# thunguyenphuoc/RenderNet

Hardware: AMD Instinct MI355X
Metric: rendered frames/sec, 64^3 voxel->512x512 Phong, batch 24 (higher is better)
Workload: dtype f32 (multiply stages: bf16x3-split operands, fp32 accumulate); 1 GPU; Phong shader forward (resampler + RenderNet 1-ch head), 5 shipped binvox fixtures cycled, 64^3 -> 128^3 -> 512x512, seeded random weights (237.3M params); batch_per_gpu=24, global_batch=24

## Files before the change

### include/rendernet_hip.h

```cpp
#ifndef RENDERNET_HIP_H
#define RENDERNET_HIP_H

#include <stddef.h>
#include <stdint.h>

#ifdef __cplusplus
extern "C" {
#endif

#define RN_VERSION 193

#define RN_OK              0
#define RN_E_INVALID      -1
#define RN_E_LAUNCH       -2
#define RN_E_UNSUPPORTED  -3

#define RN_ACT_NONE     0
#define RN_ACT_PRELU    1
#define RN_ACT_SIGMOID  2
#define RN_ACT_ELU      4

#define RN_PACK_CONV        0
#define RN_PACK_CONVT_S1    1
#define RN_PACK_CONVT_S2    2
// ... 82 lines not shown
int rn_winograd_input_transform(int scheme, const float* x, float* V, int B, int H, int W, int C, int pad_lo, void* stream);
int rn_winograd_gemm(int scheme, const float* V, const float* w_packed, float* M, long long T, int Cin, int Cout, void* stream);
int rn_winograd_output_transform(int scheme, const float* M, const float* bias, const float* alpha, const float* residual,
                                 float* y, float* preact, int B, int H, int W, int C, int act, void* stream);
#define RN_SPLIT_FMT_H2 0x100
int rn_winograd_split_supported(int scheme, int Cin, int Cout);
size_t rn_winograd_split_packed_bytes(int scheme, int Cin, int Cout);
size_t rn_winograd_split_v_bytes(int scheme, long long T, int Cin);
size_t rn_winograd_split_workspace_bytes(int scheme, int B, int H, int W, int Cin, int Cout);
int rn_winograd_split_pack(int scheme, const float* w_tf, void* w_split, int Cin, int Cout, int transposed, void* stream);
int rn_winograd_split_input_transform(int scheme, const float* x, void* Vs, int B, int H, int W, int C, int pad_lo, void* stream);
int rn_winograd_split_gemm(int scheme, const void* Vs, const void* w_split, float* M, long long T, int Cin, int Cout, void* stream);
int rn_conv2d_winograd_split_fwd(int scheme, const float* x, const void* w_split, const float* bias, const float* alpha,
                                 const float* residual, float* y, float* preact, void* workspace, int B, int H, int W,
                                 int Cin, int Cout, int transposed, int act, void* stream);
int rn_conv2d_winograd_split_fwd_ex(int scheme, const float* x, const void* w_split, const float* bias, const float* alpha,
                                    const float* residual, float* y, float* preact, void* workspace, int B, int H, int W,
                                    int Cin, int Cout, int transposed, int act, const void* amax_x, void* amax_y, void* stream);
int rn_winograd_split_input_transform_ex(int scheme, const float* x, void* Vs, int B, int H, int W, int C, int pad_lo,
                                         const void* amax_x, void* stream);
int rn_winograd_output_transform_ex(int scheme, const float* M, const float* bias, const float* alpha, const float* residual,
                                    float* y, float* preact, int B, int H, int W, int C, int act, void* amax_y, void* stream);
int rn_absmax(const float* x, long long n, void* amax, void* stream);
int rn_winograd_split_wgrad_supported(int scheme, int Cin, int Cout);
size_t rn_winograd_split_wgrad_workspace_bytes(int scheme, int B, int H, int W, int Cin, int Cout);
int rn_conv2d_winograd_split_wgrad(int scheme, const float* x, const float* dz, float* dw, void* workspace, int B, int H, int W,
                                   int Cin, int Cout, void* stream);
int rn_conv3d_winograd_split_supported(int Cin, int Cout);
size_t rn_conv3d_winograd_split_packed_bytes(int Cin, int Cout);
int rn_conv3d_winograd_split_pack(const float* w_tf, void* w_split, int Cin, int Cout, int transposed, void* stream);
int rn_conv3d_winograd_split_fwd(const float* x, const void* w_split, const float* bias, const float* alpha, const float* residual,
                                 float* y, float* preact, int B, int H, int W, int D, int Cin, int Cout, int act, void* stream);
size_t rn_conv3d_winograd_split_packed_bytes_ex(int fmt, int Cin, int Cout);
int rn_conv3d_winograd_split_pack_ex(int fmt, const float* w_tf, void* w_split, int Cin, int Cout, int transposed, void* stream);
int rn_conv3d_winograd_split_fwd_ex(int fmt, const float* x, const void* w_split, const float* bias, const float* alpha, const float* residual,
                                    float* y, float* preact, int B, int H, int W, int D, int Cin, int Cout, int act,
                                    const void* amax_x, void* amax_scratch, void* amax_y, void* stream);
int rn_conv3d_wino_supported(int Cin, int Cout);
int rn_conv2d_wino4_supported(int Cin, int Cout);
int rn_conv2d_wino4_fwd(const float* x, const float* w_wino4, const float* bias, const float* alpha,
                        const float* residual, float* y, float* preact,
                        int B, int H, int W, int Cin, int Cout, int transposed, int act, void* stream);

int rn_conv2d_transpose_s2_wino_supported(int Cin, int Cout);
int rn_conv2d_transpose_s2_wino_fwd(const float* x, const float* w_wino_s2, const float* bias, const float* alpha,
                                    const float* residual, float* y, float* preact,
// ... 171 lines not shown
```

### rendernet_amd/_lib.py

```python
import ctypes
import os

_HERE = os.path.dirname(os.path.abspath(__file__))
LIB_PATH = os.environ.get("RN_HIP_LIBRARY") or os.path.join(_HERE, "lib", "librendernet_hip.so")

RN_ACT_NONE, RN_ACT_PRELU, RN_ACT_SIGMOID, RN_ACT_ELU = 0, 1, 2, 4
RN_PHONG_NP_BLACK, RN_PHONG_NP_WHITE, RN_PHONG_TF_BLACK, RN_PHONG_TF_WHITE, RN_PHONG_NO_MASK = 0, 1, 2, 3, 4
RN_PACK_CONV, RN_PACK_CONVT_S1, RN_PACK_CONVT_S2, RN_PACK_CONV_WINO, RN_PACK_CONVT_S1_WINO = 0, 1, 2, 3, 4
RN_PACK_CONV_WINO4, RN_PACK_CONVT_S1_WINO4 = 5, 6
RN_PACK_CONV_WINO43, RN_PACK_CONVT_S1_WINO43 = 7, 8
RN_PACK_CONV_WINO44, RN_PACK_CONVT_S1_WINO44 = 9, 10
RN_PACK_CONV_WINO63, RN_PACK_CONVT_S1_WINO63 = 11, 12
RN_PACK_CONVT_S2_WINO = 13
RN_WINO_F43, RN_WINO_F44, RN_WINO_F63, RN_WINO_F11 = 0, 1, 2, 3
RN_SHAPES_MAX_PRIMS, RN_SHAPES_NOOP = 8, 255
RN_METRICS_U8, RN_METRICS_F32 = 0, 1
RN_SPLIT_FMT_H2 = 0x100

_c_int, _c_vp, _c_f = ctypes.c_int, ctypes.c_void_p, ctypes.c_float
_ip = ctypes.POINTER(ctypes.c_int)

SIGNATURES = {
    "rn_version": (_c_int, []),
    "rn_last_error": (ctypes.c_char_p, []),
# ... 42 lines not shown
    "rn_conv2d_wino43_workspace_floats": (ctypes.c_size_t, [_c_int] * 5),
    "rn_conv2d_wino43_fwd": (_c_int, [_c_vp] * 8 + [_c_int] * 6 + [_c_vp]),
    "rn_conv2d_wino63_supported": (_c_int, [_c_int, _c_int]),
    "rn_conv2d_wino63_workspace_floats": (ctypes.c_size_t, [_c_int] * 5),
    "rn_conv2d_wino63_fwd": (_c_int, [_c_vp] * 8 + [_c_int] * 6 + [_c_vp]),
    "rn_conv2d_wino44_supported": (_c_int, [_c_int, _c_int]),
    "rn_conv2d_wino44_workspace_floats": (ctypes.c_size_t, [_c_int] * 5),
    "rn_conv2d_wino44_fwd": (_c_int, [_c_vp] * 8 + [_c_int] * 7 + [_c_vp]),
    "rn_winograd_input_transform": (_c_int, [_c_int, _c_vp, _c_vp] + [_c_int] * 5 + [_c_vp]),
    "rn_winograd_gemm": (_c_int, [_c_int] + [_c_vp] * 3 + [ctypes.c_longlong, _c_int, _c_int, _c_vp]),
    "rn_winograd_output_transform": (_c_int, [_c_int] + [_c_vp] * 6 + [_c_int] * 5 + [_c_vp]),
    "rn_winograd_split_supported": (_c_int, [_c_int] * 3),
    "rn_winograd_split_packed_bytes": (ctypes.c_size_t, [_c_int] * 3),
    "rn_winograd_split_v_bytes": (ctypes.c_size_t, [_c_int, ctypes.c_longlong, _c_int]),
    "rn_winograd_split_workspace_bytes": (ctypes.c_size_t, [_c_int] * 6),
    "rn_winograd_split_pack": (_c_int, [_c_int, _c_vp, _c_vp, _c_int, _c_int, _c_int, _c_vp]),
    "rn_winograd_split_input_transform": (_c_int, [_c_int, _c_vp, _c_vp] + [_c_int] * 5 + [_c_vp]),
    "rn_winograd_split_gemm": (_c_int, [_c_int] + [_c_vp] * 3 + [ctypes.c_longlong, _c_int, _c_int, _c_vp]),
    "rn_conv2d_winograd_split_fwd": (_c_int, [_c_int] + [_c_vp] * 8 + [_c_int] * 7 + [_c_vp]),
    "rn_conv2d_winograd_split_fwd_ex": (_c_int, [_c_int] + [_c_vp] * 8 + [_c_int] * 7 + [_c_vp] * 3),
    "rn_winograd_split_input_transform_ex": (_c_int, [_c_int, _c_vp, _c_vp] + [_c_int] * 5 + [_c_vp, _c_vp]),
    "rn_winograd_output_transform_ex": (_c_int, [_c_int] + [_c_vp] * 6 + [_c_int] * 5 + [_c_vp, _c_vp]),
    "rn_absmax": (_c_int, [_c_vp, ctypes.c_longlong, _c_vp, _c_vp]),
    "rn_winograd_split_wgrad_supported": (_c_int, [_c_int, _c_int, _c_int]),
    "rn_winograd_split_wgrad_workspace_bytes": (ctypes.c_size_t, [_c_int] * 6),
    "rn_conv2d_winograd_split_wgrad": (_c_int, [_c_int] + [_c_vp] * 4 + [_c_int] * 5 + [_c_vp]),
    "rn_conv3d_winograd_split_supported": (_c_int, [_c_int, _c_int]),
    "rn_conv3d_winograd_split_packed_bytes_ex": (ctypes.c_size_t, [_c_int, _c_int, _c_int]),
    "rn_conv3d_winograd_split_pack_ex": (_c_int, [_c_int, _c_vp, _c_vp, _c_int, _c_int, _c_int, _c_vp]),
    "rn_conv3d_winograd_split_fwd_ex": (_c_int, [_c_int] + [_c_vp] * 7 + [_c_int] * 7 + [_c_vp] * 4),
    "rn_conv3d_winograd_split_packed_bytes": (ctypes.c_size_t, [_c_int, _c_int]),
    "rn_conv3d_winograd_split_pack": (_c_int, [_c_vp, _c_vp, _c_int, _c_int, _c_int, _c_vp]),
    "rn_conv3d_winograd_split_fwd": (_c_int, [_c_vp] * 7 + [_c_int] * 7 + [_c_vp]),
    "rn_conv2d_wino43_wgrad_supported": (_c_int, [_c_int, _c_int]),
    "rn_conv2d_wino43_wgrad_workspace_floats": (ctypes.c_size_t, [_c_int] * 5),
    "rn_conv2d_wino43_wgrad": (_c_int, [_c_vp] * 4 + [_c_int] * 5 + [_c_vp]),
    "rn_conv2d_wino44_wgrad_supported": (_c_int, [_c_int, _c_int]),
    "rn_conv2d_wino44_wgrad_workspace_floats": (ctypes.c_size_t, [_c_int] * 5),
    "rn_conv2d_wino44_wgrad": (_c_int, [_c_vp] * 4 + [_c_int] * 5 + [_c_vp]),
    "rn_conv2d_wino_wgrad_supported": (_c_int, [_c_int, _c_int]),
    "rn_conv2d_wino_wgrad": (_c_int, [_c_vp] * 3 + [_c_int] * 5 + [_c_vp]),
    "rn_conv2d_transpose_wgrad": (_c_int, [_c_vp] * 3 + [_c_int] * 7 + [_c_vp]),
    "rn_conv3d_transpose_wgrad": (_c_int, [_c_vp] * 3 + [_c_int] * 8 + [_c_vp]),
    "rn_resample_affine_bwd": (_c_int, [_c_vp] * 5 + [_c_int] * 9 + [_c_vp]),
    "rn_pose_to_affine_bwd": (_c_int, [_c_vp] * 3 + [_c_int] * 3 + [_c_vp]),
    "rn_dropout": (_c_int, [_c_vp, _c_vp, ctypes.c_size_t, _c_f, ctypes.c_uint64, ctypes.c_uint64, _c_vp]),
# ... 49 lines not shown

def check(rc, what=""):
    if rc != 0:
        msg = lib().rn_last_error()
        raise RenderNetHipError("%s failed (rc=%d): %s" % (what, rc, msg.decode() if msg else ""))


def ivec(vals):
    return (ctypes.c_int * len(vals))(*[int(v) for v in vals])


def ptr(t):
    if t is None:
        return None
    if not t.is_cuda:
        raise RenderNetHipError("expected a CUDA/HIP tensor, got device %s" % t.device)
    if _F32[0] is None:
        lib()
    if t.dtype is not _F32[0] or not t.is_contiguous():
        raise RenderNetHipError("expected a contiguous float32 tensor")
    return ctypes.c_void_p(t.data_ptr())


def stream_ptr():
    import torch
    return ctypes.c_void_p(torch.cuda.current_stream().cuda_stream)
```

### rendernet_amd/csrc/capi.hip

```cpp
#include "rn_common.h"
#include <stdarg.h>
#include <stdio.h>

static thread_local char g_err[512] = "";

int rn_set_error(int code, const char* fmt, ...)
{
    va_list ap;
    va_start(ap, fmt);
    vsnprintf(g_err, sizeof(g_err), fmt, ap);
    va_end(ap);
    return code;
}

int rn_check_launch(const char* what)
{
    hipError_t e = hipGetLastError();
    if (e != hipSuccess) return rn_set_error(RN_E_LAUNCH, "%s: %s", what, hipGetErrorString(e));
    return RN_OK;
}

int rn_ensure_dynamic_lds(const void* kernel, size_t bytes)
{
    struct Slot { const void* k; int dev; size_t bytes; };
// ... 417 lines not shown
}
extern "C" size_t rn_winograd_split_workspace_bytes(int scheme, int B, int H, int W, int Cin, int Cout)
{
    if (B < 1 || H < 1 || W < 1 || !rn_wino_bf3_supported(scheme, Cin, Cout)) return 0;
    return rn_wino_bf3_workspace_bytes(scheme, B, H, W, Cin, Cout);
}
extern "C" int rn_winograd_split_pack(int scheme, const float* w_tf, void* w_split, int Cin, int Cout, int transposed, void* stream)
{
    if (!w_tf || !w_split) return rn_set_error(RN_E_INVALID, "rn_winograd_split_pack: null pointer");
    return rn_launch_wino_pack_bf3(scheme, w_tf, w_split, Cin, Cout, transposed ? 1 : 0, (hipStream_t)stream);
}
extern "C" int rn_winograd_split_input_transform(int scheme, const float* x, void* Vs, int B, int H, int W, int C, int pad_lo, void* stream)
{
    if (!x || !Vs) return rn_set_error(RN_E_INVALID, "rn_winograd_split_input_transform: null pointer");
    if (rn_split_scheme_nxi(scheme & 0xff) == 0 || (scheme >> 8) > 1 || B < 1 || H < 1 || W < 1 || C < 32 || C % 32 != 0 || pad_lo < 0 || pad_lo > 3)
        return rn_set_error(RN_E_INVALID, "rn_winograd_split_input_transform: bad arguments (C must be a multiple of 32: the GEMM stage's K contract)");
    return rn_launch_wino_input_bf3(scheme, x, Vs, B, H, W, C, pad_lo, (hipStream_t)stream);
}
extern "C" int rn_winograd_split_gemm(int scheme, const void* Vs, const void* w_split, float* M, long long T, int Cin, int Cout, void* stream)
{
    if (!Vs || !w_split || !M) return rn_set_error(RN_E_INVALID, "rn_winograd_split_gemm: null pointer");
    return rn_launch_wino_gemm_bf3(scheme, Vs, w_split, M, T, Cin, Cout, (hipStream_t)stream);
}
extern "C" int rn_conv2d_winograd_split_fwd(int scheme, const float* x, const void* w_split, const float* bias, const float* alpha,
                                            const float* residual, float* y, float* preact, void* workspace, int B, int H, int W,
                                            int Cin, int Cout, int transposed, int act, void* stream)
{
    if (!x || !w_split || !y || !workspace) return rn_set_error(RN_E_INVALID, "rn_conv2d_winograd_split_fwd: null pointer");
    if (B < 1 || H < 1 || W < 1) return rn_set_error(RN_E_INVALID, "rn_conv2d_winograd_split_fwd: bad sizes");
    if ((act & RN_ACT_PRELU) && !alpha) return rn_set_error(RN_E_INVALID, "rn_conv2d_winograd_split_fwd: PReLU needs alpha");
    const int pad_lo = (scheme & 0xff) == RN_WINO_F11 ? 0 : ((scheme & 0xff) == RN_WINO_F44 && transposed) ? 2 : 1;
    return rn_launch_conv_wino_bf3(scheme, x, w_split, bias, alpha, residual, y, preact, workspace, B, H, W, Cin, Cout, pad_lo, act,
                                   (hipStream_t)stream);
}

extern "C" int rn_conv2d_winograd_split_fwd_ex(int scheme, const float* x, const void* w_split, const float* bias, const float* alpha,
                                               const float* residual, float* y, float* preact, void* workspace, int B, int H, int W,
                                               int Cin, int Cout, int transposed, int act, const void* amax_x, void* amax_y, void* stream)
{
    if (!x || !w_split || !y || !workspace) return rn_set_error(RN_E_INVALID, "rn_conv2d_winograd_split_fwd_ex: null pointer");
    if (B < 1 || H < 1 || W < 1) return rn_set_error(RN_E_INVALID, "rn_conv2d_winograd_split_fwd_ex: bad sizes");
    if ((act & RN_ACT_PRELU) && !alpha) return rn_set_error(RN_E_INVALID, "rn_conv2d_winograd_split_fwd_ex: PReLU needs alpha");
    const int pad_lo = (scheme & 0xff) == RN_WINO_F11 ? 0 : ((scheme & 0xff) == RN_WINO_F44 && transposed) ? 2 : 1;
    return rn_launch_conv_wino_bf3_ex(scheme, x, w_split, bias, alpha, residual, y, preact, workspace, B, H, W, Cin, Cout, pad_lo, act,
                                      static_cast<const unsigned*>(amax_x), static_cast<unsigned*>(amax_y), (hipStream_t)stream);
}
// ... 182 lines not shown
```

### rendernet_amd/csrc/conv_wino43.hip

```cpp
#include "wino_xform.h"
#include <stdlib.h>

namespace {

constexpr int GBM = 256, GBN = 256, GBK = 32;
constexpr int G_UB = GBK * GBN * 4;

__device__ __forceinline__ f32x4 ld4(const float* p) { return *reinterpret_cast<const f32x4*>(p); }
__device__ __forceinline__ void st4(float* p, f32x4 v) { *reinterpret_cast<f32x4*>(p) = v; }

}

template <class S, int VW>
__global__ __launch_bounds__(256)
void wino_input_kernel(const float* __restrict__ x, float* __restrict__ V, int H, int W, int C, int th, int tw,
                       long long T, unsigned nblk8, int pad_lo)
{
    typedef float vec __attribute__((ext_vector_type(VW)));
    constexpr int A = S::TA;
    const unsigned blk = xcd_contiguous(blockIdx.x, nblk8);
    const long long idx = (long long)blk * 256 + threadIdx.x;
    const int CV = C / VW;
    const int cv = (int)(idx % CV);
    const long long t = idx / CV;
    if (t >= T) return;
    vec tt[A][A];
    wino_input_btd<S, BT_DENSE>(x, t, true, cv * VW, H, W, C, th, tw, pad_lo, tt);
    float* vb = V + (size_t)t * C + cv * VW;
    const size_t plane = (size_t)T * C;
#pragma unroll
    for (int i = 0; i < A; ++i) {
        vec vrow[A];
        bt_apply<S, BT_DENSE>(tt[i], vrow);
#pragma unroll
        for (int j = 0; j < A; ++j) *reinterpret_cast<vec*>(vb + (size_t)(i * A + j) * plane) = vrow[j];
    }
}

template <class S, int VW, bool RES = false>
__global__ __launch_bounds__(256)
void wino_output_kernel(const float* __restrict__ M, const float* __restrict__ bias, const float* __restrict__ alpha,
                        const float* __restrict__ res, float* __restrict__ y, float* __restrict__ z,
                        int H, int W, int C, int th, int tw, long long T, int act, unsigned nblk8, unsigned* __restrict__ amax)
{
    typedef float vec __attribute__((ext_vector_type(VW)));
    constexpr int A = S::TA;
    const unsigned blk = xcd_contiguous(blockIdx.x, nblk8);
    const long long idx = (long long)blk * 256 + threadIdx.x;
    const int CV = C / VW;
    const int cv = (int)(idx % CV);
    const long long t_raw = idx / CV;
    if (t_raw >= T && !amax) return;
    const bool live = t_raw < T;
    const long long t = live ? t_raw : T - 1;
    float ymax = 0.f;
    const int tx = (int)(t % tw), ty = (int)((t / tw) % th);
    const long long b = t / ((long long)tw * th);
    const float* mb = M + (size_t)t * C + cv * VW;
    const size_t plane = (size_t)T * C;
    constexpr int MO = S::M;
    vec s[MO][A];
#pragma unroll
    for (int j = 0; j < A; ++j) {
        vec m[A];
#pragma unroll
        for (int i = 0; i < A; ++i) m[i] = __builtin_nontemporal_load(reinterpret_cast<const vec*>(mb + (size_t)(i * A + j) * plane));
#pragma unroll
        for (int p_ = 0; p_ < MO; ++p_) {
            vec acc = vec(0.f);
#pragma unroll
            for (int i = 0; i < A; ++i) {
                const float c = S::AT(p_, i);
                if (c != 0.f) acc += c * m[i];
            }
            s[p_][j] = acc;
        }
    }
// ... 357 lines not shown
    if (ragged > 0) {
        a.mb_begin = full; a.mblocks = 1;
        const int nitems = nxi * a.nblocks;
        int best_wm = 4, best_parts = 1, best_cost = (nitems + 255) / 256 * 4;
        for (int wm = 2; wm >= 1; --wm) {
            const int parts = (ragged + wm * 64 - 1) / (wm * 64);
            const int cost = (nitems * parts + 255) / 256 * wm;
            if (cost < best_cost) { best_wm = wm; best_parts = parts; best_cost = cost; }
        }
        return wino43_gemm_launch(best_wm, tag, a, 0, nitems, best_parts, st);
    }
    return RN_OK;
}

int rn_launch_wino_output(int scheme, const float* M, const float* bias, const float* alpha, const float* residual, float* y,
                          float* preact, int B, int H, int W, int C, int act, hipStream_t st)
{
    return rn_launch_wino_output_amax(scheme, M, bias, alpha, residual, y, preact, B, H, W, C, act, nullptr, st);
}

int rn_launch_wino_output_amax(int scheme, const float* M, const float* bias, const float* alpha, const float* residual, float* y,
                               float* preact, int B, int H, int W, int C, int act, unsigned* amax, hipStream_t st)
{
    const int m = rn_split_scheme_m(scheme);
    if (m == 0) return rn_set_error(RN_E_INVALID, "wino_output: unknown scheme %d", scheme);
    const int th = (H + m - 1) / m, tw = (W + m - 1) / m;
    const long long T = (long long)B * th * tw;
    if (!wino_with_scheme<WINO_SPLIT>(scheme, [&](auto s) {
            typedef decltype(s) S;
            constexpr int VW = wino_vw<S>;
            const unsigned long long n = ((unsigned long long)T * (C / VW) + 255) / 256;
            const unsigned nblk8 = (unsigned)((n + 7) / 8 * 8);
            if (residual) hipLaunchKernelGGL((wino_output_kernel<S, VW, true>), dim3(nblk8), dim3(256), 0, st, M, bias, alpha, residual, y, preact,
                                             H, W, C, th, tw, T, act, nblk8, amax);
            else hipLaunchKernelGGL((wino_output_kernel<S, VW, false>), dim3(nblk8), dim3(256), 0, st, M, bias, alpha, residual, y, preact,
                                    H, W, C, th, tw, T, act, nblk8, amax);
        }))
        return rn_set_error(RN_E_INVALID, "wino_output: unknown scheme %d", scheme);
    return rn_check_launch("wino_output");
}

long long rn_wino43_plane_limit()
{
    const char* e = getenv("RN_WINO43_MAX_PLANE");
    const long long v = e ? atoll(e) : 0;
    return (v > 0 && v < 0x7fffff00LL) ? v : 0x7fffff00LL;
}

size_t rn_wino43_workspace_floats(int scheme, int B, int H, int W, int Cin, int Cout)
{
    const int m = rn_wino_scheme_m(scheme);
    if (m == 0) return 0;
    const size_t T = (size_t)B * ((H + m - 1) / m) * ((W + m - 1) / m);
    return (size_t)rn_wino_scheme_nxi(scheme) * T * ((size_t)Cin + Cout);
}

int rn_launch_conv_wino43(int scheme, const float* x, const float* u, const float* bias, const float* alpha, const float* residual,
                          float* y, float* preact, float* ws, int B, int H, int W, int Cin, int Cout, int pad_lo, int act, hipStream_t st)
{
// ... 28 lines not shown
```

### rendernet_amd/csrc/conv_wino_bf3.hip

```cpp
#include "wino_xform.h"
#include <stdlib.h>

#ifndef RN_BF3_M_AUX
#define RN_BF3_M_AUX 0
#endif
#ifndef RN_BF3_VLOAD_AUX
#define RN_BF3_VLOAD_AUX 0
#endif
#ifndef RN_BF3_ULOAD_AUX
#define RN_BF3_ULOAD_AUX 0
#endif
#ifndef RN_BF3_VSTORE_NT
#define RN_BF3_VSTORE_NT 0
#endif

using rnf::FmtB3;
using rnf::FmtH2;

namespace {
constexpr int SB_ROW = 96;
constexpr int SB_BM = 256, SB_BN = 256;
constexpr int SB_NSTAGE = 3;
}

// ... 666 lines not shown
    hipLaunchKernelGGL(kern, dim3(n < 256 ? (unsigned)((n + 7) / 8 * 8) : 256u), dim3(512), lds, st, a);
    return rn_check_launch("wino_gemm_bf3");
}

template <class F, int WM>
static int wino_gemm_bf3_launch_w(int tag, const Bf3GemmArgs& a, int begin, int end, int parts, hipStream_t st)
{
    switch (tag) {
    case 0: return wino_gemm_bf3_launch_t<F, WM, 0>(a, begin, end, parts, st);
    case 1: return wino_gemm_bf3_launch_t<F, WM, 1>(a, begin, end, parts, st);
    case 2: return wino_gemm_bf3_launch_t<F, WM, 2>(a, begin, end, parts, st);
    case 4: return wino_gemm_bf3_launch_t<F, WM, 4>(a, begin, end, parts, st);
    case 5: return wino_gemm_bf3_launch_t<F, WM, 5>(a, begin, end, parts, st);
    default: return wino_gemm_bf3_launch_t<F, WM, 3>(a, begin, end, parts, st);
    }
}

static int wino_gemm_bf3_launch(int fmt, int wm, int tag, const Bf3GemmArgs& a, int begin, int end, int parts, hipStream_t st)
{
    if (fmt == 1) return wm == 4 ? wino_gemm_bf3_launch_w<FmtH2, 4>(tag, a, begin, end, parts, st) : wino_gemm_bf3_launch_w<FmtH2, 2>(tag, a, begin, end, parts, st);
    return wm == 4 ? wino_gemm_bf3_launch_w<FmtB3, 4>(tag, a, begin, end, parts, st) : wino_gemm_bf3_launch_w<FmtB3, 2>(tag, a, begin, end, parts, st);
}

static int gemm_split_planes(int fmt, int nxi, int tag, const void* Vs, const void* us, float* M, long long T, int Cin, int Cout,
                             const unsigned* amax_v, const unsigned* amax_u, float bound_v, float bound_u, hipStream_t st)
{
    const int SB_ROW = fmt == 1 ? FmtH2::ROW : FmtB3::ROW;
    if (nxi < 1 || Cin < 16 || Cin % 16 != 0 || Cout < SB_BN || Cout % SB_BN != 0)
        return rn_set_error(RN_E_UNSUPPORTED, "gemm_bf3: planes=%d K=%d N=%d", nxi, Cin, Cout);
    if (T < 1 || (T + SB_BM) * (long long)Cout * 4 >= 0xffffff00LL || T * (long long)Cout * 4 >= 0x7fffff00LL || (T + SB_BM) * (long long)SB_ROW >= 0x7fffff00LL)
        return rn_set_error(RN_E_UNSUPPORTED, "wino_gemm_bf3: a transform plane must stay below the 2 GiB buffer window");
    Bf3GemmArgs a;
    a.V = static_cast<const char*>(Vs); a.U = static_cast<const char*>(us); a.M = M; a.T = T; a.Cin = Cin; a.Cout = Cout;
    a.nblocks = Cout / SB_BN; a.ksteps = Cin / 16;
    a.v_step_bytes = (unsigned)(T * SB_ROW); a.m_bytes = (unsigned)(T * Cout * 4);
    a.amax_v = amax_v; a.amax_u = amax_u; a.bound_v = bound_v; a.bound_u = bound_u;
    static const bool notail = getenv("RN_WINO_BF3_NOTAIL") != nullptr;
    const int full = (int)(T / SB_BM), ragged = (int)(T % SB_BM);
    if ((long long)nxi * (full + 1) * a.nblocks * 2 > 0x3fffffff) return rn_set_error(RN_E_UNSUPPORTED, "wino_gemm_bf3: too many items");
    a.mrows = SB_BM;
    static const int HC = getenv("RN_WINO_BF3_HALF_COST") ? atoi(getenv("RN_WINO_BF3_HALF_COST")) : 9;
    constexpr int WC = 16, LC = 4;
    auto tail_cost = [](int rem) { if (rem == 0) return 0; const int half = (2 * rem + 255) / 256; return half < 2 ? half * HC : WC; };
    auto ragged_plan = [&](int& wm, int& parts) {
        const int nit = nxi * a.nblocks;
        wm = 4; parts = 1;
        int best = (nit + 255) / 256 * WC;
        const int hp = (ragged + 127) / 128, hc = (nit * hp + 255) / 256 * HC;
        if (!notail && hc < best) { best = hc; wm = 2; parts = hp; }
        return best;
    };
    if (!notail && full <= 1) {
        const int nfull = nxi * full * a.nblocks;
        const int tc = tail_cost(nfull % 256);
        int cost_split = nfull / 256 * WC + tc, launches = (nfull >= 256 || tc == WC) + (tc != 0 && tc < WC);
        if (ragged > 0) { int wm, parts; cost_split += ragged_plan(wm, parts); ++launches; }
        cost_split += LC * (launches - 1);
        if (ragged > 0 && full == 1) {
            const int nm = nxi * 2 * a.nblocks, tcm = tail_cost(nm % 256);
            const int merged = nm / 256 * WC + tcm + (tcm != 0 && tcm < WC && nm >= 256 ? LC : 0);
            if (merged < cost_split) cost_split = merged;
        }
        const long long items = (long long)nxi * a.nblocks * ((T + 127) / 128);
        const int ucost = (int)((items + 255) / 256) * HC;
        if (ucost <= cost_split) {
            a.mb_begin = 0; a.mrows = 128; a.mblocks = (int)((T + 127) / 128);
            return wino_gemm_bf3_launch(fmt, 2, tag, a, 0, nxi * a.mblocks * a.nblocks, 1, st);
        }
    }
    auto main_cost = [&](int nitems) {
        const int rem = nitems % 256, tc = tail_cost(rem);
        return nitems / 256 * WC + tc + (tc != 0 && tc < WC && nitems >= 256 ? LC : 0);
    };
    static const bool nomerge = getenv("RN_WINO_BF3_NOMERGE") != nullptr;
    int blocks = full, left = ragged;
    if (ragged > 0 && !notail && !nomerge) {
        int wm, parts;
        const int separate = main_cost(nxi * full * a.nblocks) + ragged_plan(wm, parts) + (full > 0 ? LC : 0);
        if (main_cost(nxi * (full + 1) * a.nblocks) < separate) { blocks = full + 1; left = 0; }
    }
    if (blocks > 0) {
        a.mb_begin = 0; a.mblocks = blocks;
        const int nitems = nxi * blocks * a.nblocks;
        const int rem = nitems % 256;
        const bool half_tail = !notail && rem != 0 && tail_cost(rem) < WC;
        const int tail = half_tail ? rem : 0;
        if (nitems - tail > 0) {
            const int rc = wino_gemm_bf3_launch(fmt, 4, tag, a, 0, nitems - tail, 0, st);
            if (rc != RN_OK) return rc;
        }
        if (tail > 0) {
            const int rc = wino_gemm_bf3_launch(fmt, 2, tag, a, nitems - tail, nitems, 0, st);
            if (rc != RN_OK) return rc;
        }
    }
    if (left > 0) {
        a.mb_begin = full; a.mblocks = 1;
        int wm, parts;
        ragged_plan(wm, parts);
        return wino_gemm_bf3_launch(fmt, wm, tag, a, 0, nxi * a.nblocks, parts, st);
    }
    return RN_OK;
}

int rn_launch_gemm_bf3_planes(int nxi, int tag, const void* Vs, const void* us, float* M, long long T, int Cin, int Cout, hipStream_t st)
{
    return gemm_split_planes(0, nxi, tag, Vs, us, M, T, Cin, Cout, nullptr, nullptr, 1.f, 1.f, st);
}

int rn_launch_wino_gemm_bf3(int scheme, const void* Vs, const void* us, float* M, long long T, int Cin, int Cout, hipStream_t st)
{
    if (!rn_wino_bf3_supported(scheme, Cin, Cout)) return rn_set_error(RN_E_UNSUPPORTED, "wino_gemm_bf3: scheme=%d Cin=%d Cout=%d", scheme, Cin, Cout);
    const int fmt = fmt_of(scheme);
    scheme = sch_of(scheme);
    const int tag = scheme == RN_WINO_F11 ? 5 : scheme == RN_WINO_F43 ? 0 : scheme == RN_WINO_F44 ? 1 : Cin >= 1024 ? 2 : 3;
    if (fmt == 1) {
        const unsigned* av = reinterpret_cast<const unsigned*>(static_cast<const char*>(Vs) + h2_v_data(scheme, T, Cin));
        const unsigned* au = reinterpret_cast<const unsigned*>(static_cast<const char*>(us) + h2_u_data(scheme, Cin, Cout));
        return gemm_split_planes(1, rn_split_scheme_nxi(scheme), tag, Vs, us, M, T, Cin, Cout, av, au, h2_bound_v(scheme), h2_bound_u(scheme), st);
    }
    return rn_launch_gemm_bf3_planes(rn_split_scheme_nxi(scheme), tag, Vs, us, M, T, Cin, Cout, st);
}

int rn_launch_conv_wino_bf3(int scheme, const float* x, const void* us, const float* bias, const float* alpha, const float* residual,
                            float* y, float* preact, void* ws, int B, int H, int W, int Cin, int Cout, int pad_lo, int act, hipStream_t st)
{
    return rn_launch_conv_wino_bf3_ex(scheme, x, us, bias, alpha, residual, y, preact, ws, B, H, W, Cin, Cout, pad_lo, act, nullptr, nullptr, st);
}

static int conv_wino_bf3_rec(int scheme, const float* x, const void* us, const float* bias, const float* alpha, const float* residual,
                             float* y, float* preact, void* ws, int B, int H, int W, int Cin, int Cout, int pad_lo, int act,
                             const unsigned* amax_x, unsigned* amax_y, hipStream_t st)
{
    const int m = rn_split_scheme_m(sch_of(scheme));
    const int th = (H + m - 1) / m, tw = (W + m - 1) / m;
    const long long T = (long long)B * th * tw;
    const int cmax = Cin > Cout ? Cin : Cout;
    const long long lim = rn_wino43_plane_limit();
    if ((long long)th * tw * cmax * 4 >= lim)
        return rn_set_error(RN_E_UNSUPPORTED, "conv_wino_bf3: one image's transform plane exceeds the 2 GiB buffer window");
    if (T * cmax * 4 >= lim) {
        const int chunk = (int)((lim - 1) / ((long long)th * tw * cmax * 4));
        for (int b0 = 0; b0 < B; b0 += chunk) {
            const int nb = B - b0 < chunk ? B - b0 : chunk;
            const size_t xo = (size_t)b0 * H * W * Cin, yo = (size_t)b0 * H * W * Cout;
            const int rc = conv_wino_bf3_rec(scheme, x + xo, us, bias, alpha, residual ? residual + yo : nullptr, y + yo,
                                             preact ? preact + yo : nullptr, ws, nb, H, W, Cin, Cout, pad_lo, act, amax_x, amax_y, st);
            if (rc != RN_OK) return rc;
        }
        return RN_OK;
    }
    char* Vs = static_cast<char*>(ws);
    float* M = reinterpret_cast<float*>(Vs + rn_wino_bf3_v_bytes(scheme, T, Cin));
    int rc = rn_launch_wino_input_bf3_ex(scheme, x, Vs, B, H, W, Cin, pad_lo, amax_x, st);
    if (rc != RN_OK) return rc;
    rc = rn_launch_wino_gemm_bf3(scheme, Vs, us, M, T, Cin, Cout, st);
    if (rc != RN_OK) return rc;
    return rn_launch_wino_output_amax(sch_of(scheme), M, bias, alpha, residual, y, preact, B, H, W, Cout, act, amax_y, st);
}

int rn_launch_conv_wino_bf3_ex(int scheme, const float* x, const void* us, const float* bias, const float* alpha, const float* residual,
                               float* y, float* preact, void* ws, int B, int H, int W, int Cin, int Cout, int pad_lo, int act,
                               const unsigned* amax_x, unsigned* amax_y, hipStream_t st)
{
    if (!rn_wino_bf3_supported(scheme, Cin, Cout)) return rn_set_error(RN_E_UNSUPPORTED, "conv_wino_bf3: scheme=%d Cin=%d Cout=%d", scheme, Cin, Cout);
    if (amax_y) { const int rc = rn_launch_word(amax_y, nullptr, st); if (rc != RN_OK) return rc; }
    return conv_wino_bf3_rec(scheme, x, us, bias, alpha, residual, y, preact, ws, B, H, W, Cin, Cout, pad_lo, act, amax_x, amax_y, st);
}
```

### rendernet_amd/csrc/rn_common.h

```cpp
#pragma once
#include <hip/hip_runtime.h>
#include <stdint.h>
#include <stddef.h>
#include "../../include/rendernet_hip.h"

struct RnConvProblem {
    const float* x;
    const float* w;
    const float* bias;
    const float* alpha;
    const float* residual;
    float* y;
    float* preact;
    int B, I[3], Cin;
    int O[3], Cout, Npad;
    int K[3], S[3], P[3];
    long long os_b, os[3], out_off;
    int act;
};

int rn_set_error(int code, const char* fmt, ...);
int rn_check_launch(const char* what);

int rn_launch_conv_igemm(const RnConvProblem& p, hipStream_t st);
// ... 12 lines not shown
                        int mode, int pad, hipStream_t st);

struct WinoF11 {
    static constexpr int M = 1, TA = 1, R = 1, NXI = 1;
    static constexpr float AT(int, int) { return 1.f; }
    static constexpr double G(int, int) { return 1.0; }
    static constexpr float BT(int, int) { return 1.f; }
};
int rn_split_scheme_nxi(int scheme);
int rn_split_scheme_m(int scheme);
bool rn_wino43_supported(int scheme, int Cin, int Cout);
int rn_wino_scheme_nxi(int scheme);
int rn_wino_scheme_r(int scheme);
int rn_wino_scheme_m(int scheme);
long long rn_wino43_plane_limit();
size_t rn_wino43_workspace_floats(int scheme, int B, int H, int W, int Cin, int Cout);
int rn_launch_wino_pack(int scheme, const float* w_tf, float* u, int Cin, int Cout, int transposed, hipStream_t st);
int rn_launch_wino_input(int scheme, const float* x, float* V, int B, int H, int W, int C, int pad_lo, hipStream_t st);
int rn_launch_wino_gemm(int scheme, const float* V, const float* u, float* M, long long T, int Cin, int Cout, hipStream_t st);
int rn_launch_wino_output(int scheme, const float* M, const float* bias, const float* alpha, const float* residual, float* y,
                          float* preact, int B, int H, int W, int C, int act, hipStream_t st);
int rn_launch_wino_output_amax(int scheme, const float* M, const float* bias, const float* alpha, const float* residual, float* y,
                               float* preact, int B, int H, int W, int C, int act, unsigned* amax, hipStream_t st);
int rn_launch_conv_wino43(int scheme, const float* x, const float* u, const float* bias, const float* alpha, const float* residual,
                          float* y, float* preact, float* ws, int B, int H, int W, int Cin, int Cout, int pad_lo, int act, hipStream_t st);
bool rn_wino_bf3_supported(int scheme, int Cin, int Cout);
size_t rn_wino_bf3_packed_bytes(int scheme, int Cin, int Cout);
size_t rn_wino_bf3_v_bytes(int scheme, long long T, int Cin);
size_t rn_wino_bf3_workspace_bytes(int scheme, int B, int H, int W, int Cin, int Cout);
int rn_launch_wino_pack_bf3(int scheme, const float* w_tf, void* us, int Cin, int Cout, int transposed, hipStream_t st);
int rn_launch_wino_input_bf3(int scheme, const float* x, void* Vs, int B, int H, int W, int C, int pad_lo, hipStream_t st);
int rn_launch_word(unsigned* dst, const unsigned* src, hipStream_t st);
int rn_launch_absmax(const float* x, size_t n, unsigned* out, hipStream_t st);
int rn_launch_wino_input_bf3_ex(int scheme, const float* x, void* Vs, int B, int H, int W, int C, int pad_lo, const unsigned* amax_x, hipStream_t st);
int rn_launch_conv_wino_bf3_ex(int scheme, const float* x, const void* us, const float* bias, const float* alpha, const float* residual,
                               float* y, float* preact, void* ws, int B, int H, int W, int Cin, int Cout, int pad_lo, int act,
                               const unsigned* amax_x, unsigned* amax_y, hipStream_t st);
int rn_launch_wino_gemm_bf3(int scheme, const void* Vs, const void* us, float* M, long long T, int Cin, int Cout, hipStream_t st);
int rn_launch_gemm_bf3_planes(int nplanes, int tag, const void* Vs, const void* us, float* M, long long T, int Cin, int Cout, hipStream_t st);
bool rn_wino_bf3_wgrad_supported(int scheme, int Cin, int Cout);
size_t rn_wino_bf3_wgrad_workspace_bytes(int scheme, int B, int H, int W, int Cin, int Cout);
int rn_launch_conv_wino_bf3_wgrad(int scheme, const float* x, const float* dz, float* dw, void* ws, int B, int H, int W, int Cin, int Cout, hipStream_t st);
int rn_launch_conv_wino_bf3(int scheme, const float* x, const void* us, const float* bias, const float* alpha, const float* residual,
                            float* y, float* preact, void* ws, int B, int H, int W, int Cin, int Cout, int pad_lo, int act, hipStream_t st);
bool rn_conv3d_wino_bf3_supported(int Cin, int Cout);
size_t rn_conv3d_wino_bf3_packed_bytes();
int rn_launch_conv3d_wino_pack_bf3(const float* w_tf, void* us, int transposed, hipStream_t st);
int rn_launch_conv3d_wino_bf3(const float* x, const void* us, const float* bias, const float* alpha, const float* residual,
                              float* y, float* preact, int B, int H, int W, int D, int act, hipStream_t st);
size_t rn_conv3d_wino_split_packed_bytes(int fmt);
int rn_launch_conv3d_wino_split_pack(int fmt, const float* w_tf, void* us, int transposed, hipStream_t st);
int rn_launch_conv3d_wino_split(int fmt, const float* x, const void* us, const float* bias, const float* alpha, const float* residual,
                                float* y, float* preact, int B, int H, int W, int D, int act, const unsigned* amax_x, unsigned* scratch_amax,
                                unsigned* amax_y, hipStream_t st);
bool rn_wino43_wgrad_supported(int scheme, int Cin, int Cout);
size_t rn_wino43_wgrad_workspace_floats(int scheme, int B, int H, int W, int Cin, int Cout);
int rn_launch_conv_wino43_wgrad(int scheme, const float* x, const float* dz, float* dw, float* ws, int B, int H, int W, int Cin, int Cout, hipStream_t st);
bool rn_wino_wgrad_supported(int Cin, int Cout);
int rn_launch_conv_wino_wgrad(const float* x, const float* dz, float* dw, int B, int H, int W, int Cin, int Cout, hipStream_t st);

bool rn_conv3d_wgrad_split_ok(int Cin, int Cout);
// ... 15 lines not shown
```

Baseline: 329.8 frames/s.

## Overlap ragged Winograd GEMM tail with output transform on a side stream

Splits the bf16x3 Winograd conv so the ragged last M-block of the split GEMM runs on a dedicated non-blocking side stream. Meanwhile the main stream runs the output transform for the whole tiles, then joins and transforms the ragged tiles. A dry-run plan mode of the GEMM launcher detects when a ragged block exists. The aim is to hide the under-occupied tail launch behind the output transform, at the cost of extra event record/wait overhead, a mutex, and an extra output-transform launch. It is skipped under graph capture.

```diff
diff --git a/include/rendernet_hip.h b/include/rendernet_hip.h
--- a/include/rendernet_hip.h
+++ b/include/rendernet_hip.h
@@ -128,6 +128,10 @@
 int rn_winograd_output_transform_ex(int scheme, const float* M, const float* bias, const float* alpha, const float* residual,
                                     float* y, float* preact, int B, int H, int W, int C, int act, void* amax_y, void* stream);
 int rn_absmax(const float* x, long long n, void* amax, void* stream);
+void rn_set_wino_tail_overlap(int on);
+int rn_get_wino_tail_overlap(void);
+long long rn_get_wino_tail_overlap_forks(void);
+int rn_winograd_split_gemm_plan(int scheme, long long T, int Cin, int Cout, int* launches, int* ragged_rows);
 int rn_winograd_split_wgrad_supported(int scheme, int Cin, int Cout);
 size_t rn_winograd_split_wgrad_workspace_bytes(int scheme, int B, int H, int W, int Cin, int Cout);
 int rn_conv2d_winograd_split_wgrad(int scheme, const float* x, const float* dz, float* dw, void* workspace, int B, int H, int W,
diff --git a/rendernet_amd/_lib.py b/rendernet_amd/_lib.py
--- a/rendernet_amd/_lib.py
+++ b/rendernet_amd/_lib.py
@@ -88,6 +88,10 @@
     "rn_winograd_split_input_transform_ex": (_c_int, [_c_int, _c_vp, _c_vp] + [_c_int] * 5 + [_c_vp, _c_vp]),
     "rn_winograd_output_transform_ex": (_c_int, [_c_int] + [_c_vp] * 6 + [_c_int] * 5 + [_c_vp, _c_vp]),
     "rn_absmax": (_c_int, [_c_vp, ctypes.c_longlong, _c_vp, _c_vp]),
+    "rn_set_wino_tail_overlap": (None, [_c_int]),
+    "rn_get_wino_tail_overlap": (_c_int, []),
+    "rn_get_wino_tail_overlap_forks": (ctypes.c_longlong, []),
+    "rn_winograd_split_gemm_plan": (_c_int, [_c_int, ctypes.c_longlong, _c_int, _c_int, _ip, _ip]),
     "rn_winograd_split_wgrad_supported": (_c_int, [_c_int, _c_int, _c_int]),
     "rn_winograd_split_wgrad_workspace_bytes": (ctypes.c_size_t, [_c_int] * 6),
     "rn_conv2d_winograd_split_wgrad": (_c_int, [_c_int] + [_c_vp] * 4 + [_c_int] * 5 + [_c_vp]),
@@ -183,6 +187,12 @@
     return ctypes.c_void_p(t.data_ptr())
 
 
+def split_gemm_plan(scheme, T, Cin, Cout):
+    n, r = ctypes.c_int(0), ctypes.c_int(0)
+    check(lib().rn_winograd_split_gemm_plan(scheme, T, Cin, Cout, ctypes.byref(n), ctypes.byref(r)), "rn_winograd_split_gemm_plan")
+    return n.value, r.value
+
+
 def stream_ptr():
     import torch
     return ctypes.c_void_p(torch.cuda.current_stream().cuda_stream)
diff --git a/rendernet_amd/csrc/capi.hip b/rendernet_amd/csrc/capi.hip
--- a/rendernet_amd/csrc/capi.hip
+++ b/rendernet_amd/csrc/capi.hip
@@ -463,6 +463,13 @@
     if (!Vs || !w_split || !M) return rn_set_error(RN_E_INVALID, "rn_winograd_split_gemm: null pointer");
     return rn_launch_wino_gemm_bf3(scheme, Vs, w_split, M, T, Cin, Cout, (hipStream_t)stream);
 }
+extern "C" int rn_winograd_split_gemm_plan(int scheme, long long T, int Cin, int Cout, int* launches, int* ragged_rows)
+{
+    return rn_wino_gemm_bf3_plan(scheme, T, Cin, Cout, launches, ragged_rows);
+}
+extern "C" void rn_set_wino_tail_overlap(int on) { rn_wino_tail_overlap_set(on); }
+extern "C" int rn_get_wino_tail_overlap(void) { return rn_wino_tail_overlap_get(); }
+extern "C" long long rn_get_wino_tail_overlap_forks(void) { return rn_wino_tail_overlap_forks(); }
 extern "C" int rn_conv2d_winograd_split_fwd(int scheme, const float* x, const void* w_split, const float* bias, const float* alpha,
                                             const float* residual, float* y, float* preact, void* workspace, int B, int H, int W,
                                             int Cin, int Cout, int transposed, int act, void* stream)
diff --git a/rendernet_amd/csrc/conv_wino43.hip b/rendernet_amd/csrc/conv_wino43.hip
--- a/rendernet_amd/csrc/conv_wino43.hip
+++ b/rendernet_amd/csrc/conv_wino43.hip
@@ -41,7 +41,8 @@
 __global__ __launch_bounds__(256)
 void wino_output_kernel(const float* __restrict__ M, const float* __restrict__ bias, const float* __restrict__ alpha,
                         const float* __restrict__ res, float* __restrict__ y, float* __restrict__ z,
-                        int H, int W, int C, int th, int tw, long long T, int act, unsigned nblk8, unsigned* __restrict__ amax)
+                        int H, int W, int C, int th, int tw, long long T, int act, unsigned nblk8, unsigned* __restrict__ amax,
+                        long long t_begin, long long t_end)
 {
     typedef float vec __attribute__((ext_vector_type(VW)));
     constexpr int A = S::TA;
@@ -49,10 +50,10 @@
     const long long idx = (long long)blk * 256 + threadIdx.x;
     const int CV = C / VW;
     const int cv = (int)(idx % CV);
-    const long long t_raw = idx / CV;
-    if (t_raw >= T && !amax) return;
-    const bool live = t_raw < T;
-    const long long t = live ? t_raw : T - 1;
+    const long long t_raw = t_begin + idx / CV;
+    if (t_raw >= t_end && !amax) return;
+    const bool live = t_raw < t_end;
+    const long long t = live ? t_raw : t_end - 1;
     float ymax = 0.f;
     const int tx = (int)(t % tw), ty = (int)((t / tw) % th);
     const long long b = t / ((long long)tw * th);
@@ -456,19 +457,28 @@
 int rn_launch_wino_output_amax(int scheme, const float* M, const float* bias, const float* alpha, const float* residual, float* y,
                                float* preact, int B, int H, int W, int C, int act, unsigned* amax, hipStream_t st)
 {
+    return rn_launch_wino_output_range(scheme, M, bias, alpha, residual, y, preact, B, H, W, C, act, amax, 0, -1, st);
+}
+
+int rn_launch_wino_output_range(int scheme, const float* M, const float* bias, const float* alpha, const float* residual, float* y,
+                                float* preact, int B, int H, int W, int C, int act, unsigned* amax, long long t_begin, long long t_end,
+                                hipStream_t st)
+{
     const int m = rn_split_scheme_m(scheme);
     if (m == 0) return rn_set_error(RN_E_INVALID, "wino_output: unknown scheme %d", scheme);
     const int th = (H + m - 1) / m, tw = (W + m - 1) / m;
     const long long T = (long long)B * th * tw;
+    if (t_end < 0) t_end = T;
+    if (t_begin < 0 || t_begin >= t_end || t_end > T) return rn_set_error(RN_E_INVALID, "wino_output: tiles [%lld, %lld) of %lld", t_begin, t_end, T);
     if (!wino_with_scheme<WINO_SPLIT>(scheme, [&](auto s) {
             typedef decltype(s) S;
             constexpr int VW = wino_vw<S>;
-            const unsigned long long n = ((unsigned long long)T * (C / VW) + 255) / 256;
+            const unsigned long long n = ((unsigned long long)(t_end - t_begin) * (C / VW) + 255) / 256;
             const unsigned nblk8 = (unsigned)((n + 7) / 8 * 8);
             if (residual) hipLaunchKernelGGL((wino_output_kernel<S, VW, true>), dim3(nblk8), dim3(256), 0, st, M, bias, alpha, residual, y, preact,
-                                             H, W, C, th, tw, T, act, nblk8, amax);
+                                             H, W, C, th, tw, T, act, nblk8, amax, t_begin, t_end);
             else hipLaunchKernelGGL((wino_output_kernel<S, VW, false>), dim3(nblk8), dim3(256), 0, st, M, bias, alpha, residual, y, preact,
-                                    H, W, C, th, tw, T, act, nblk8, amax);
+                                    H, W, C, th, tw, T, act, nblk8, amax, t_begin, t_end);
         }))
         return rn_set_error(RN_E_INVALID, "wino_output: unknown scheme %d", scheme);
     return rn_check_launch("wino_output");
diff --git a/rendernet_amd/csrc/conv_wino_bf3.hip b/rendernet_amd/csrc/conv_wino_bf3.hip
--- a/rendernet_amd/csrc/conv_wino_bf3.hip
+++ b/rendernet_amd/csrc/conv_wino_bf3.hip
@@ -1,5 +1,7 @@
 #include "wino_xform.h"
 #include <stdlib.h>
+#include <atomic>
+#include <mutex>
 
 #ifndef RN_BF3_M_AUX
 #define RN_BF3_M_AUX 0
@@ -712,9 +714,13 @@
     return wm == 4 ? wino_gemm_bf3_launch_w<FmtB3, 4>(tag, a, begin, end, parts, st) : wino_gemm_bf3_launch_w<FmtB3, 2>(tag, a, begin, end, parts, st);
 }
 
+struct SplitGemmPlan { int launches, ragged_rows; };
+
 static int gemm_split_planes(int fmt, int nxi, int tag, const void* Vs, const void* us, float* M, long long T, int Cin, int Cout,
-                             const unsigned* amax_v, const unsigned* amax_u, float bound_v, float bound_u, hipStream_t st)
-{
+                             const unsigned* amax_v, const unsigned* amax_u, float bound_v, float bound_u, hipStream_t st,
+                             hipStream_t ragged_st = nullptr, SplitGemmPlan* plan = nullptr)
+{
+    if (plan) plan->launches = plan->ragged_rows = 0;
     const int SB_ROW = fmt == 1 ? FmtH2::ROW : FmtB3::ROW;
     if (nxi < 1 || Cin < 16 || Cin % 16 != 0 || Cout < SB_BN || Cout % SB_BN != 0)
         return rn_set_error(RN_E_UNSUPPORTED, "gemm_bf3: planes=%d K=%d N=%d", nxi, Cin, Cout);
@@ -729,6 +735,10 @@
     const int full = (int)(T / SB_BM), ragged = (int)(T % SB_BM);
     if ((long long)nxi * (full + 1) * a.nblocks * 2 > 0x3fffffff) return rn_set_error(RN_E_UNSUPPORTED, "wino_gemm_bf3: too many items");
     a.mrows = SB_BM;
+    auto launch = [&](int wm, int begin, int end, int parts, hipStream_t s) {
+        if (plan) { ++plan->launches; return (int)RN_OK; }
+        return wino_gemm_bf3_launch(fmt, wm, tag, a, begin, end, parts, s);
+    };
     static const int HC = getenv("RN_WINO_BF3_HALF_COST") ? atoi(getenv("RN_WINO_BF3_HALF_COST")) : 9;
     constexpr int WC = 16, LC = 4;
     auto tail_cost = [](int rem) { if (rem == 0) return 0; const int half = (2 * rem + 255) / 256; return half < 2 ? half * HC : WC; };
@@ -755,7 +765,7 @@
         const int ucost = (int)((items + 255) / 256) * HC;
         if (ucost <= cost_split) {
             a.mb_begin = 0; a.mrows = 128; a.mblocks = (int)((T + 127) / 128);
-            return wino_gemm_bf3_launch(fmt, 2, tag, a, 0, nxi * a.mblocks * a.nblocks, 1, st);
+            return launch(2, 0, nxi * a.mblocks * a.nblocks, 1, st);
         }
     }
     auto main_cost = [&](int nitems) {
@@ -776,11 +786,11 @@
         const bool half_tail = !notail && rem != 0 && tail_cost(rem) < WC;
         const int tail = half_tail ? rem : 0;
         if (nitems - tail > 0) {
-            const int rc = wino_gemm_bf3_launch(fmt, 4, tag, a, 0, nitems - tail, 0, st);
+            const int rc = launch(4, 0, nitems - tail, 0, st);
             if (rc != RN_OK) return rc;
         }
         if (tail > 0) {
-            const int rc = wino_gemm_bf3_launch(fmt, 2, tag, a, nitems - tail, nitems, 0, st);
+            const int rc = launch(2, nitems - tail, nitems, 0, st);
             if (rc != RN_OK) return rc;
         }
     }
@@ -788,7 +798,8 @@
         a.mb_begin = full; a.mblocks = 1;
         int wm, parts;
         ragged_plan(wm, parts);
-        return wino_gemm_bf3_launch(fmt, wm, tag, a, 0, nxi * a.nblocks, parts, st);
+        if (plan && full >= 1) plan->ragged_rows = left;
+        return launch(wm, 0, nxi * a.nblocks, parts, full >= 1 && ragged_st ? ragged_st : st);
     }
     return RN_OK;
 }
@@ -798,18 +809,74 @@
     return gemm_split_planes(0, nxi, tag, Vs, us, M, T, Cin, Cout, nullptr, nullptr, 1.f, 1.f, st);
 }
 
-int rn_launch_wino_gemm_bf3(int scheme, const void* Vs, const void* us, float* M, long long T, int Cin, int Cout, hipStream_t st)
+static int wino_gemm_split(int scheme, const void* Vs, const void* us, float* M, long long T, int Cin, int Cout, hipStream_t st,
+                           hipStream_t ragged_st, SplitGemmPlan* plan)
 {
     if (!rn_wino_bf3_supported(scheme, Cin, Cout)) return rn_set_error(RN_E_UNSUPPORTED, "wino_gemm_bf3: scheme=%d Cin=%d Cout=%d", scheme, Cin, Cout);
     const int fmt = fmt_of(scheme);
     scheme = sch_of(scheme);
     const int tag = scheme == RN_WINO_F11 ? 5 : scheme == RN_WINO_F43 ? 0 : scheme == RN_WINO_F44 ? 1 : Cin >= 1024 ? 2 : 3;
     if (fmt == 1) {
-        const unsigned* av = reinterpret_cast<const unsigned*>(static_cast<const char*>(Vs) + h2_v_data(scheme, T, Cin));
-        const unsigned* au = reinterpret_cast<const unsigned*>(static_cast<const char*>(us) + h2_u_data(scheme, Cin, Cout));
-        return gemm_split_planes(1, rn_split_scheme_nxi(scheme), tag, Vs, us, M, T, Cin, Cout, av, au, h2_bound_v(scheme), h2_bound_u(scheme), st);
-    }
-    return rn_launch_gemm_bf3_planes(rn_split_scheme_nxi(scheme), tag, Vs, us, M, T, Cin, Cout, st);
+        const unsigned* av = plan ? nullptr : reinterpret_cast<const unsigned*>(static_cast<const char*>(Vs) + h2_v_data(scheme, T, Cin));
+        const unsigned* au = plan ? nullptr : reinterpret_cast<const unsigned*>(static_cast<const char*>(us) + h2_u_data(scheme, Cin, Cout));
+        return gemm_split_planes(1, rn_split_scheme_nxi(scheme), tag, Vs, us, M, T, Cin, Cout, av, au, h2_bound_v(scheme), h2_bound_u(scheme), st, ragged_st, plan);
+    }
+    return gemm_split_planes(0, rn_split_scheme_nxi(scheme), tag, Vs, us, M, T, Cin, Cout, nullptr, nullptr, 1.f, 1.f, st, ragged_st, plan);
+}
+
+int rn_launch_wino_gemm_bf3(int scheme, const void* Vs, const void* us, float* M, long long T, int Cin, int Cout, hipStream_t st)
+{
+    return wino_gemm_split(scheme, Vs, us, M, T, Cin, Cout, st, nullptr, nullptr);
+}
+
+int rn_wino_gemm_bf3_plan(int scheme, long long T, int Cin, int Cout, int* launches, int* ragged_rows)
+{
+    SplitGemmPlan p;
+    const int rc = wino_gemm_split(scheme, nullptr, nullptr, nullptr, T, Cin, Cout, nullptr, nullptr, &p);
+    if (rc != RN_OK) return rc;
+    if (launches) *launches = p.launches;
+    if (ragged_rows) *ragged_rows = p.ragged_rows;
+    return RN_OK;
+}
+
+namespace {
+struct TailSide { hipStream_t st = nullptr; hipEvent_t fork = nullptr, join = nullptr; bool failed = false; };
+constexpr int MAX_DEV = 64;
+TailSide g_tail_side[MAX_DEV];
+std::mutex g_tail_mutex;
+std::atomic<int> g_tail_overlap{-1};
+std::atomic<long long> g_tail_forks{0};
+
+TailSide* tail_side()
+{
+    int dev = -1;
+    if (hipGetDevice(&dev) != hipSuccess || dev < 0 || dev >= MAX_DEV) { (void)hipGetLastError(); return nullptr; }
+    TailSide& s = g_tail_side[dev];
+    if (s.failed) return nullptr;
+    if (!s.st) {
+        if (hipStreamCreateWithFlags(&s.st, hipStreamNonBlocking) != hipSuccess || hipEventCreateWithFlags(&s.fork, hipEventDisableTiming) != hipSuccess
+            || hipEventCreateWithFlags(&s.join, hipEventDisableTiming) != hipSuccess) {
+            (void)hipGetLastError();
+            s.failed = true; s.st = nullptr;
+            return nullptr;
+        }
+    }
+    return &s;
+}
+}
+
+void rn_wino_tail_overlap_set(int on) { g_tail_overlap.store(on ? 1 : 0); }
+long long rn_wino_tail_overlap_forks() { return g_tail_forks.load(); }
+int rn_wino_tail_overlap_get()
+{
+    int v = g_tail_overlap.load();
+    if (v < 0) {
+        const char* e = getenv("RN_WINO_TAIL_OVERLAP");
+        v = (e && atoi(e) == 0 && e[0] != '\0') ? 0 : 1;
+        int expect = -1;
+        if (!g_tail_overlap.compare_exchange_strong(expect, v)) v = expect;
+    }
+    return v;
 }
 
 int rn_launch_conv_wino_bf3(int scheme, const float* x, const void* us, const float* bias, const float* alpha, const float* residual,
@@ -844,6 +911,31 @@
     float* M = reinterpret_cast<float*>(Vs + rn_wino_bf3_v_bytes(scheme, T, Cin));
     int rc = rn_launch_wino_input_bf3_ex(scheme, x, Vs, B, H, W, Cin, pad_lo, amax_x, st);
     if (rc != RN_OK) return rc;
+    SplitGemmPlan plan = {0, 0};
+    if (rn_wino_tail_overlap_get() && wino_gemm_split(scheme, nullptr, nullptr, nullptr, T, Cin, Cout, nullptr, nullptr, &plan) == RN_OK && plan.ragged_rows > 0) {
+        hipStreamCaptureStatus cap = hipStreamCaptureStatusNone;
+        if (hipStreamIsCapturing(st, &cap) != hipSuccess) { (void)hipGetLastError(); cap = hipStreamCaptureStatusActive; }
+        if (cap == hipStreamCaptureStatusNone) {
+            std::lock_guard<std::mutex> lock(g_tail_mutex);
+            TailSide* side = tail_side();
+            if (side && hipEventRecord(side->fork, st) == hipSuccess && hipStreamWaitEvent(side->st, side->fork, 0) == hipSuccess) {
+                const long long t_whole = T - plan.ragged_rows;
+                ++g_tail_forks;
+                rc = wino_gemm_split(scheme, Vs, us, M, T, Cin, Cout, st, side->st, nullptr);
+                if (rc == RN_OK)
+                    rc = rn_launch_wino_output_range(sch_of(scheme), M, bias, alpha, residual, y, preact, B, H, W, Cout, act, amax_y, 0, t_whole, st);
+                if (hipEventRecord(side->join, side->st) != hipSuccess || hipStreamWaitEvent(st, side->join, 0) != hipSuccess) {
+                    (void)hipGetLastError();
+                    (void)hipStreamSynchronize(side->st);
+                    if (rc == RN_OK) rc = rn_set_error(RN_E_LAUNCH, "conv_wino_bf3: joining the ragged block's stream failed");
+                }
+                if (rc == RN_OK)
+                    rc = rn_launch_wino_output_range(sch_of(scheme), M, bias, alpha, residual, y, preact, B, H, W, Cout, act, amax_y, t_whole, T, st);
+                return rc;
+            }
+            (void)hipGetLastError();
+        }
+    }
     rc = rn_launch_wino_gemm_bf3(scheme, Vs, us, M, T, Cin, Cout, st);
     if (rc != RN_OK) return rc;
     return rn_launch_wino_output_amax(sch_of(scheme), M, bias, alpha, residual, y, preact, B, H, W, Cout, act, amax_y, st);
diff --git a/rendernet_amd/csrc/rn_common.h b/rendernet_amd/csrc/rn_common.h
--- a/rendernet_amd/csrc/rn_common.h
+++ b/rendernet_amd/csrc/rn_common.h
@@ -58,6 +58,9 @@
                           float* preact, int B, int H, int W, int C, int act, hipStream_t st);
 int rn_launch_wino_output_amax(int scheme, const float* M, const float* bias, const float* alpha, const float* residual, float* y,
                                float* preact, int B, int H, int W, int C, int act, unsigned* amax, hipStream_t st);
+int rn_launch_wino_output_range(int scheme, const float* M, const float* bias, const float* alpha, const float* residual, float* y,
+                                float* preact, int B, int H, int W, int C, int act, unsigned* amax, long long t_begin, long long t_end,
+                                hipStream_t st);
 int rn_launch_conv_wino43(int scheme, const float* x, const float* u, const float* bias, const float* alpha, const float* residual,
                           float* y, float* preact, float* ws, int B, int H, int W, int Cin, int Cout, int pad_lo, int act, hipStream_t st);
 bool rn_wino_bf3_supported(int scheme, int Cin, int Cout);
@@ -73,6 +76,10 @@
                                float* y, float* preact, void* ws, int B, int H, int W, int Cin, int Cout, int pad_lo, int act,
                                const unsigned* amax_x, unsigned* amax_y, hipStream_t st);
 int rn_launch_wino_gemm_bf3(int scheme, const void* Vs, const void* us, float* M, long long T, int Cin, int Cout, hipStream_t st);
+int rn_wino_gemm_bf3_plan(int scheme, long long T, int Cin, int Cout, int* launches, int* ragged_rows);
+void rn_wino_tail_overlap_set(int on);
+int rn_wino_tail_overlap_get();
+long long rn_wino_tail_overlap_forks();
 int rn_launch_gemm_bf3_planes(int nplanes, int tag, const void* Vs, const void* us, float* M, long long T, int Cin, int Cout, hipStream_t st);
 bool rn_wino_bf3_wgrad_supported(int scheme, int Cin, int Cout);
 size_t rn_wino_bf3_wgrad_workspace_bytes(int scheme, int B, int H, int W, int Cin, int Cout);
```

New measurement: 330.7 frames/s (median of 6 runs). No clear change (+0.3%).
